# VITA-Group/mm-hand

Measured on AMD Instinct MI355X. Metric: 256x256 hand images/sec (G+D step), higher is better.
Workload: dtype f32; 1 GPU; RHD-shaped 256x256, per-GPU batch 32, fp32 (Winograd F(6x6,3x3) on the 3x3 stack), G(9 PATBlocks, ngf64)+D_PB+D_PP+L1/perceptual/GAN+Adam, --norm instance, dropout on; VGG19[:4] weights: random-init (seed 1234): NOT the reference's pretrained objective; global_batch=32, parallelism=dp1

## Files before the change

### mmhand_amd/csrc/common.h

```cpp
#pragma once
#include <hip/hip_runtime.h>
#include <cstdarg>
#include <cstdio>
#include <cstdint>
#include "../../include/mmhand_hip.h"

namespace mmh {

char* err_buf();
int fail(const char* fmt, ...);

inline int check_launch(const char* what) {
    hipError_t e = hipGetLastError();
    if (e != hipSuccess) return fail("%s: %s", what, hipGetErrorString(e));
    return 0;
}

inline hipStream_t as_stream(mmh_stream_t s) { return reinterpret_cast<hipStream_t>(s); }

inline int64_t cdiv(int64_t a, int64_t b) { return (a + b - 1) / b; }

int wino6_weights(const float* w, float* U, int Cin, int Cout, int flip_transpose, hipStream_t st);
int wino6_weights_multi(const long long* table, int n, long long total_blocks, hipStream_t st);
int wino6_input(const float* x, float* V, int B, int H, int W, int C, int reflect, int xcd, hipStream_t st);
int wino6_output(const float* M, float* y, const float* bias, int B, int H, int W, int C, int act, float* stats,
                 int fold, hipStream_t st);
int wino6_dy(const float* dy, float* Yh, int B, int H, int W, int C, hipStream_t st);
int wino6_input_normact(const float* x, float* V, int B, int H, int W, int C, int reflect, int xcd,
                        const float* scale, const float* shift, int groups, int relu, float drop_p,
                        const uint32_t* drows, hipStream_t st);
int wino6_input_dy_normbwd(const float* g, const float* x, float* V, float* Yh, int B, int H, int W, int C, int xcd,
                           int fold, const float* mean, const float* invstd, const float* gamma, const float* s1,
                           const float* s2, double count, const float* scale, const float* shift,
                           const uint32_t* drows, int groups, int relu, float drop_p, hipStream_t st);
int wino6_input_dy(const float* dy, float* V, float* Yh, int B, int H, int W, int C, int xcd, int fold,
                   hipStream_t st);
int wino6_dw(const float* dU, float* dw, int Cin, int Cout, int accumulate, hipStream_t st);
bool wgrad_lp16t_supported(const mmh_conv_desc* d);
int wgrad_lp16t_splits(const mmh_conv_desc* d);
int launch_wgrad_lp16t(const mmh_conv_desc* d, const void* x16, const void* dy16, float* slab, const void* zeros,
                       hipStream_t st);
bool dgrad_s2_halo_ok(const mmh_conv_desc* d, int dx_cs, int act);
int launch_dgrad_s2_halo(const mmh_conv_desc* d, const void* dy, const void* w, const void* bias, void* dx, int dx_cs,
                         int act, hipStream_t st);
extern int g_dgrad_s2_halo, g_dgrad_s2_dbg;
bool wgrad_s2_strip_ok(const mmh_conv_desc* d);
size_t wgrad_s2_strip_ws_bytes(const mmh_conv_desc* d);
int launch_wgrad_s2_strip(const mmh_conv_desc* d, const void* x, const void* dy, void* dw, void* ws, size_t ws_bytes,
                          int accumulate, hipStream_t st);
extern int g_wgrad_s2_strip;
bool stem_f32_ok(const mmh_conv_desc* d);
int stem_f32_stats_chunks(const mmh_conv_desc* d);
int launch_stem_f32(const mmh_conv_desc* d, const void* x, const void* w, const void* bias, void* y, int act, float* stats,
                    hipStream_t st);
extern int g_stem_f32, g_stem_f32_dbg, g_stem_f32_levels;
extern int g_stem_sparse;
extern int g_stem_sparse_flat;
void wgrad_flat_split(int Mrows, int N, int P, int& splits, int& pix_per_split);
bool wino_wgrad_dma_ok(int64_t tiles, int Cin, int Cout, int nbatch);
size_t wino_wgrad_dma_ws_bytes(int64_t tiles, int Cin, int Cout, int nbatch);
int launch_wino_wgrad_dma(const float* V, const float* Yh, int64_t tiles, int Cin, int Cout, int nbatch, float* ws, float* dU,
                          hipStream_t st);
extern int g_wino_wgrad_dma;
int launch_slab_reduce(const float* slab, float* dw, int64_t n4_total, int splits, int accumulate, int64_t n4, hipStream_t st);
bool conv_s2f_ok(const mmh_conv_desc* d, int mode);
bool conv_s1f_ok(const mmh_conv_desc* d, int mode);
int conv_s2f_stats_chunks(const mmh_conv_desc* d);
int launch_conv_s2f(const mmh_conv_desc* d, const void* x16, const void* w16, const void* bias, void* y, int y_is16, int act,
                    const void* zeros, hipStream_t st, float* stats = nullptr, int mode = 0);
bool conv_s2d_ok(const mmh_conv_desc* d, int mode);
int launch_conv_s2d(const mmh_conv_desc* d, const void* g16, const void* w16, const void* bias, void* dx, int dx_is16, int act,
                    const void* zeros, hipStream_t st);
extern int g_lp16_s2f;
extern int g_lp16_persist;
extern int g_slab_reduce_par;
extern int g_wino6_vec;
extern int g_lp16_shape;
extern int g_lp16_tap_inner;
extern int g_lp16_dbg;
extern int g_lp16_wgrad_ring;
extern int g_lp16_wgrad_s2;
extern int g_pw_v2;
extern int g_col_chunks, g_row_chunks;

}

#define MMH_REQUIRE(cond, ...)                      \
    do {                                            \
        if (!(cond)) return mmh::fail(__VA_ARGS__); \
    } while (0)
```

### mmhand_amd/csrc/conv_igemm.hip

```cpp
#include <algorithm>
#include <cstring>
#include "device_prims.h"

namespace {
using namespace mmh::dev;

typedef __bf16 bf16x4 __attribute__((ext_vector_type(4)));
typedef __bf16 bf16x2 __attribute__((ext_vector_type(2)));
typedef _Float16 f16x4 __attribute__((ext_vector_type(4)));
typedef _Float16 f16x2 __attribute__((ext_vector_type(2)));
__device__ __forceinline__ bf16x4 to_bf16x4(float4 v) {
    bf16x4 r;
    r[0] = (__bf16)v.x; r[1] = (__bf16)v.y; r[2] = (__bf16)v.z; r[3] = (__bf16)v.w;
    return r;
}
template <bool H16>
__device__ __forceinline__ bf16x4 to_lp4(float4 v) {
    if (H16) {
        f16x4 r;
        r[0] = (_Float16)v.x; r[1] = (_Float16)v.y; r[2] = (_Float16)v.z; r[3] = (_Float16)v.w;
        return __builtin_bit_cast(bf16x4, r);
    }
    return to_bf16x4(v);
}
// ... 2461 lines not shown
        wst4<BF>(Yh, (long long)(r * 4 + 2) * plane + o, f4sub(t[r][0], t[r][1]));
        wst4<BF>(Yh, (long long)(r * 4 + 3) * plane + o, f4sub(z, t[r][1]));
    }
}

__global__ void wino_dw_kernel(const float* __restrict__ dU, float* __restrict__ dw, int64_t plane4,
                               int accumulate) {
    int64_t i = (int64_t)blockIdx.x * blockDim.x + threadIdx.x;
    if (i >= plane4) return;
    const float4* in = reinterpret_cast<const float4*>(dU) + i;
    float4 u[4][4];
#pragma unroll
    for (int a = 0; a < 4; ++a)
#pragma unroll
        for (int b = 0; b < 4; ++b) u[a][b] = in[(int64_t)(a * 4 + b) * plane4];
    auto half = [](float4 v) { return make_float4(0.5f * v.x, 0.5f * v.y, 0.5f * v.z, 0.5f * v.w); };
    float4 t[3][4];
#pragma unroll
    for (int b = 0; b < 4; ++b) {
        const float4 hs = half(f4add(u[1][b], u[2][b])), hd = half(f4sub(u[1][b], u[2][b]));
        t[0][b] = f4add(u[0][b], hs);
        t[1][b] = hd;
        t[2][b] = f4add(hs, u[3][b]);
    }
    float4* out = reinterpret_cast<float4*>(dw) + i;
#pragma unroll
    for (int a = 0; a < 3; ++a) {
        const float4 hs = half(f4add(t[a][1], t[a][2])), hd = half(f4sub(t[a][1], t[a][2]));
        float4 g0 = f4add(t[a][0], hs), g1 = hd, g2 = f4add(hs, t[a][3]);
        if (accumulate) {
            g0 = f4add(g0, out[(int64_t)(a * 3 + 0) * plane4]);
            g1 = f4add(g1, out[(int64_t)(a * 3 + 1) * plane4]);
            g2 = f4add(g2, out[(int64_t)(a * 3 + 2) * plane4]);
        }
        out[(int64_t)(a * 3 + 0) * plane4] = g0;
        out[(int64_t)(a * 3 + 1) * plane4] = g1;
        out[(int64_t)(a * 3 + 2) * plane4] = g2;
    }
}

struct F2 { float x, y; };
__device__ __forceinline__ F2 operator+(F2 a, F2 b) { return {a.x + b.x, a.y + b.y}; }
__device__ __forceinline__ F2 operator-(F2 a, F2 b) { return {a.x - b.x, a.y - b.y}; }
__device__ __forceinline__ F2 operator*(float k, F2 a) { return {k * a.x, k * a.y}; }

__device__ __forceinline__ void w4_bt(const F2* in, F2* out) {
    out[0] = 4.f * in[0] - 5.f * in[2] + in[4];
    out[1] = in[3] + in[4] - 4.f * (in[1] + in[2]);
    out[2] = 4.f * (in[1] - in[2]) - in[3] + in[4];
    out[3] = 2.f * (in[3] - in[1]) - in[2] + in[4];
    out[4] = 2.f * (in[1] - in[3]) - in[2] + in[4];
    out[5] = 4.f * in[1] - 5.f * in[3] + in[5];
}
__device__ __forceinline__ void w4_at(const F2* in, F2* out) {
    const F2 a = in[1] + in[2], b = in[1] - in[2], c = in[3] + in[4], d = in[3] - in[4];
    out[0] = in[0] + a + c;
    out[1] = b + 2.f * d;
    out[2] = a + 4.f * c;
    out[3] = b + 8.f * d + in[5];
}
__device__ __forceinline__ void w4_a(const F2* in, F2* out) {
    out[0] = in[0];
    out[1] = in[0] + in[1] + in[2] + in[3];
    out[2] = in[0] - in[1] + in[2] - in[3];
    out[3] = in[0] + 2.f * in[1] + 4.f * in[2] + 8.f * in[3];
    out[4] = in[0] - 2.f * in[1] + 4.f * in[2] - 8.f * in[3];
    out[5] = in[3];
}
__device__ __forceinline__ void w4_g(const float* in, float* out) {
    out[0] = 0.25f * in[0];
    out[1] = (-1.f / 6.f) * (in[0] + in[1] + in[2]);
    out[2] = (-1.f / 6.f) * (in[0] - in[1] + in[2]);
    out[3] = (1.f / 24.f) * in[0] + (1.f / 12.f) * in[1] + (1.f / 6.f) * in[2];
    out[4] = (1.f / 24.f) * in[0] - (1.f / 12.f) * in[1] + (1.f / 6.f) * in[2];
    out[5] = in[2];
}
__device__ __forceinline__ void w4_gt(const F2* in, F2* out) {
    out[0] = 0.25f * in[0] - (1.f / 6.f) * (in[1] + in[2]) + (1.f / 24.f) * (in[3] + in[4]);
    out[1] = (1.f / 6.f) * (in[2] - in[1]) + (1.f / 12.f) * (in[3] - in[4]);
    out[2] = (1.f / 6.f) * (in[3] + in[4] - in[1] - in[2]) + in[5];
}

__global__ void wino4_weights_kernel(const float* __restrict__ w, float* __restrict__ U, int Cin, int Cout,
                                     int flip_transpose) {
    const int total = Cin * Cout;
    int i = blockIdx.x * blockDim.x + threadIdx.x;
    if (i >= total) return;
    const int ci = flip_transpose ? i % Cin : i / Cout, co = flip_transpose ? i / Cin : i - (i / Cout) * Cout;
    float g[3][3], t[6][3], col[3], o6[6];
#pragma unroll
    for (int a = 0; a < 3; ++a)
#pragma unroll
        for (int b = 0; b < 3; ++b) {
            const int ka = flip_transpose ? 2 - a : a, kb = flip_transpose ? 2 - b : b;
            g[a][b] = w[((size_t)(ka * 3 + kb) * Cin + ci) * Cout + co];
        }
#pragma unroll
    for (int b = 0; b < 3; ++b) {
        col[0] = g[0][b]; col[1] = g[1][b]; col[2] = g[2][b];
        w4_g(col, o6);
#pragma unroll
        for (int a = 0; a < 6; ++a) t[a][b] = o6[a];
    }
    const size_t plane = (size_t)Cin * Cout;
    const size_t o = flip_transpose ? (size_t)co * Cin + ci : (size_t)ci * Cout + co;
#pragma unroll
    for (int a = 0; a < 6; ++a) {
        w4_g(t[a], o6);
#pragma unroll
        for (int b = 0; b < 6; ++b) U[(size_t)(a * 6 + b) * plane + o] = o6[b];
    }
}

__global__ void wino4_input_kernel(const float* __restrict__ x, float* __restrict__ V, int B, int H, int W,
                                   int C2, int reflect, int xcd_remap) {
    const int TH = H / 4, TW = W / 4;
    const long long tiles = (long long)B * TH * TW;
    unsigned blk = blockIdx.x;
    if (xcd_remap) blk = (blk & 7u) * (gridDim.x >> 3) + (blk >> 3);
    long long i = (long long)blk * blockDim.x + threadIdx.x;
    if (i >= tiles * C2) return;
    const int c = (int)(i % C2);
    const long long tile = i / C2;
    const int tx = (int)(tile % TW), ty = (int)((tile / TW) % TH), b = (int)(tile / ((long long)TW * TH));
    const F2* xin = reinterpret_cast<const F2*>(x);
    F2 d[6][6], t[6][6], colv[6], o6[6];
#pragma unroll
    for (int r = 0; r < 6; ++r) {
        int hh = 4 * ty - 1 + r;
        bool okh = true;
        if (reflect) { hh = hh < 0 ? -hh : hh; hh = hh >= H ? 2 * (H - 1) - hh : hh; }
        else okh = hh >= 0 && hh < H;
#pragma unroll
        for (int q = 0; q < 6; ++q) {
            int ww = 4 * tx - 1 + q;
            bool ok = okh;
            if (reflect) { ww = ww < 0 ? -ww : ww; ww = ww >= W ? 2 * (W - 1) - ww : ww; }
            else ok = ok && ww >= 0 && ww < W;
            d[r][q] = ok ? xin[(((long long)b * H + hh) * W + ww) * C2 + c] : F2{0.f, 0.f};
        }
    }
#pragma unroll
    for (int q = 0; q < 6; ++q) {
#pragma unroll
        for (int r = 0; r < 6; ++r) colv[r] = d[r][q];
        w4_bt(colv, o6);
#pragma unroll
        for (int r = 0; r < 6; ++r) t[r][q] = o6[r];
    }
    const long long plane = tiles * C2;
    F2* out = reinterpret_cast<F2*>(V) + tile * C2 + c;
#pragma unroll
    for (int r = 0; r < 6; ++r) {
        w4_bt(t[r], o6);
#pragma unroll
        for (int q = 0; q < 6; ++q) out[(long long)(r * 6 + q) * plane] = o6[q];
    }
}

__global__ void wino4_output_kernel(const float* __restrict__ M, float* __restrict__ y,
                                    const float* __restrict__ bias, int B, int H, int W, int C2, int act) {
    const int TH = H / 4, TW = W / 4;
    const long long tiles = (long long)B * TH * TW;
    long long i = (long long)blockIdx.x * blockDim.x + threadIdx.x;
    if (i >= tiles * C2) return;
    const int c = (int)(i % C2);
    const long long tile = i / C2;
    const int tx = (int)(tile % TW), ty = (int)((tile / TW) % TH), b = (int)(tile / ((long long)TW * TH));
    const long long plane = tiles * C2;
    const F2* in = reinterpret_cast<const F2*>(M) + tile * C2 + c;
    F2 m[6][6], s4[4][6], colv[6], o4[4];
#pragma unroll
    for (int r = 0; r < 6; ++r)
#pragma unroll
        for (int q = 0; q < 6; ++q) m[r][q] = in[(long long)(r * 6 + q) * plane];
#pragma unroll
    for (int q = 0; q < 6; ++q) {
#pragma unroll
        for (int r = 0; r < 6; ++r) colv[r] = m[r][q];
        w4_at(colv, o4);
#pragma unroll
        for (int r = 0; r < 4; ++r) s4[r][q] = o4[r];
    }
    const F2 bv = bias ? reinterpret_cast<const F2*>(bias)[c] : F2{0.f, 0.f};
    F2* yo = reinterpret_cast<F2*>(y);
#pragma unroll
    for (int r = 0; r < 4; ++r) {
        w4_at(s4[r], o4);
#pragma unroll
        for (int q = 0; q < 4; ++q) {
            F2 v = o4[q] + bv;
            v.x = act_apply(v.x, act); v.y = act_apply(v.y, act);
            yo[(((long long)b * H + 4 * ty + r) * W + 4 * tx + q) * C2 + c] = v;
        }
    }
}

__global__ void wino4_dy_kernel(const float* __restrict__ dy, float* __restrict__ Yh, int B, int H, int W,
                                int C2) {
    const int TH = H / 4, TW = W / 4;
    const long long tiles = (long long)B * TH * TW;
    long long i = (long long)blockIdx.x * blockDim.x + threadIdx.x;
    if (i >= tiles * C2) return;
    const int c = (int)(i % C2);
    const long long tile = i / C2;
    const int tx = (int)(tile % TW), ty = (int)((tile / TW) % TH), b = (int)(tile / ((long long)TW * TH));
    const F2* in = reinterpret_cast<const F2*>(dy);
    F2 yv[4][4], t[6][4], colv[4], o6[6];
#pragma unroll
    for (int r = 0; r < 4; ++r)
#pragma unroll
        for (int q = 0; q < 4; ++q) yv[r][q] = in[(((long long)b * H + 4 * ty + r) * W + 4 * tx + q) * C2 + c];
#pragma unroll
    for (int q = 0; q < 4; ++q) {
#pragma unroll
        for (int r = 0; r < 4; ++r) colv[r] = yv[r][q];
        w4_a(colv, o6);
#pragma unroll
        for (int r = 0; r < 6; ++r) t[r][q] = o6[r];
    }
    const long long plane = tiles * C2;
    F2* out = reinterpret_cast<F2*>(Yh) + tile * C2 + c;
#pragma unroll
    for (int r = 0; r < 6; ++r) {
        w4_a(t[r], o6);
#pragma unroll
        for (int q = 0; q < 6; ++q) out[(long long)(r * 6 + q) * plane] = o6[q];
    }
}

__global__ void wino4_dw_kernel(const float* __restrict__ dU, float* __restrict__ dw, int64_t plane2,
                                int accumulate) {
    int64_t i = (int64_t)blockIdx.x * blockDim.x + threadIdx.x;
    if (i >= plane2) return;
    const F2* in = reinterpret_cast<const F2*>(dU) + i;
    F2 u[6][6], t[3][6], colv[6], o3[3];
#pragma unroll
    for (int a = 0; a < 6; ++a)
#pragma unroll
        for (int b = 0; b < 6; ++b) u[a][b] = in[(int64_t)(a * 6 + b) * plane2];
#pragma unroll
    for (int b = 0; b < 6; ++b) {
#pragma unroll
        for (int a = 0; a < 6; ++a) colv[a] = u[a][b];
        w4_gt(colv, o3);
#pragma unroll
        for (int a = 0; a < 3; ++a) t[a][b] = o3[a];
    }
    F2* out = reinterpret_cast<F2*>(dw) + i;
#pragma unroll
    for (int a = 0; a < 3; ++a) {
        w4_gt(t[a], o3);
#pragma unroll
        for (int b = 0; b < 3; ++b) {
            F2 v = o3[b];
            if (accumulate) v = v + out[(int64_t)(a * 3 + b) * plane2];
            out[(int64_t)(a * 3 + b) * plane2] = v;
        }
    }
}

template <int BN, int WM, int WN, bool NMAJOR>
int launch_batched_t(const BatchKP& bp, int nbatch, hipStream_t st) {
    constexpr size_t lds = (BM * LDA + (NMAJOR ? BN * LDA : BK * BN)) * sizeof(float) + tab_bytes(BM);
    static int ready = -1;
    if (ready != 0) ready = allow_lds(conv_igemm_batched_kernel<BN, WM, WN, NMAJOR>, lds);
    if (ready != 0) return ready;
    dim3 grid((bp.p.N + BN - 1) / BN, (bp.p.M + BM - 1) / BM, nbatch);
    hipLaunchKernelGGL((conv_igemm_batched_kernel<BN, WM, WN, NMAJOR>), grid, dim3(256), lds, st, bp);
    return mmh::check_launch("conv_igemm_batched_kernel");
}

int g_wino_bn256 = 0;
int g_wino_xcd = 1;
int g_wino_gemm_v2 = 1;
int g_wino_bf16_bk = 64;
int g_wino_bf16_occ = 3;
int g_wino_gemm_occ = 3;
int g_wino_gemm_levels = 2;
int g_wino_gemm_bn = 0;

template <int BN, int LEVELS>
static int launch_wino_gemm_t(const WinoGemmKP& p, hipStream_t st) {
    constexpr size_t lds = (size_t)(BM * LDA + BK * BN) * sizeof(float);
    static int ready = -1;
    if (ready != 0) ready = allow_lds(wino_gemm_kernel<BN, LEVELS>, lds);
    if (ready != 0) return ready;
    hipLaunchKernelGGL((wino_gemm_kernel<BN, LEVELS>), dim3(8 * p.nb), dim3(256), lds, st, p);
    return mmh::check_launch("wino_gemm_kernel");
}

static int wino_gemm_v2(const float* V, const float* U, float* Mo, long long tiles, int K, int N, hipStream_t st,
                        int nbatch, int levels, bool fold16 = false) {
    WinoGemmKP p{};
    p.A = V; p.B = U; p.C = Mo;
    p.M = (int)tiles; p.K = K; p.N = N; p.P = nbatch;
    const int bn = g_wino_gemm_bn == 64 ? 64 : (N > 64 ? 128 : 64);
    p.MT = (p.M + BM - 1) / BM;
    p.NT = (N + bn - 1) / bn;
    p.W = nbatch * p.MT * p.NT;
    p.Wx = (p.W + 7) / 8;
    const bool two = (levels ? levels : g_wino_gemm_levels) == 2 && (nbatch == 64 || fold16) && K > WINO_FOLD * BK;
    p.nb = std::min(p.Wx, 32 * g_wino_gemm_occ);
    if (two) return bn == 128 ? launch_wino_gemm_t<128, 2>(p, st) : launch_wino_gemm_t<64, 2>(p, st);
    return bn == 128 ? launch_wino_gemm_t<128, 1>(p, st) : launch_wino_gemm_t<64, 1>(p, st);
}

int wino_gemm(const float* V, const float* U, float* Mo, long long tiles, int K, int N, hipStream_t st,
              int nbatch = 16, int levels = 0) {
    MMH_REQUIRE(tiles * (long long)std::max(K, N) < (1ll << 30), "winograd: tensor too large");
    if (g_wino_gemm_v2 && K % BK == 0 && N >= 64 && N % 32 == 0) return wino_gemm_v2(V, U, Mo, tiles, K, N, st, nbatch, levels);
    BatchKP bp{};
    ConvKP& p = bp.p;
    Gather& g = p.g;
    g.src = V;
    g.src_bytes = (unsigned)((size_t)tiles * K * sizeof(float));
    g.srcH = 1; g.srcW = (int)tiles; g.src_cs = (unsigned)K;
    g.PH = 1; g.PW = (int)tiles; g.TH = 1; g.TW = 1;
    g.C4 = K / 4;
    g.ap_h = 0; g.at_h = 0; g.a0_h = 0; g.ap_w = 1; g.at_w = 0; g.a0_w = 0;
    g.shift = 0; g.reflect = 0;
    set_korder(g, p.nk, p.Kflat);
    p.w = U;
    p.w_bytes = (unsigned)((size_t)K * N * sizeof(float));
    p.out = Mo;
    p.M = (int)tiles; p.N = N;
    p.wCin = K; p.wCout = N;
    p.KW_true = 1; p.kh0 = 0; p.kw0 = 0; p.tstep = 1;
    p.OH = 1; p.OW = (int)tiles; p.o_p = 1;
    p.out_cs = (unsigned)N; p.out_linear = 1;
    p.act = MMH_ACT_NONE;
    bp.src_bs = tiles * K; bp.w_bs = (long long)K * N; bp.out_bs = tiles * N;
    {
        const int bn = (N % 256 == 0 && g_wino_bn256) ? 256 : 128;
        const int gx = (N + bn - 1) / bn, gy = (p.M + BM - 1) / BM;
        p.xcd_remap = (g_conv_xcd && gx > 1 && gy >= 8) ? 1 : 0;
    }
    if (N % 256 == 0 && g_wino_bn256) return launch_batched_t<256, 2, 2, false>(bp, nbatch, st);
    if (N > 64) return launch_batched_t<128, 2, 2, false>(bp, nbatch, st);
    if (N > 32) return launch_batched_t<64, 2, 2, false>(bp, nbatch, st);
    return launch_batched_t<32, 4, 1, false>(bp, nbatch, st);
}

int g_wgrad_slots = 768;
int g_wgrad_bn256 = 1;
int g_wino_wgrad_v2 = 1;
int g_wino_wgrad_occ = 3;
int g_wgrad_xcd = 1;
int g_wino_wgrad_bn256 = 0;
int g_wino_wgrad_slots = 2304;

int wgrad_splits(int Mrows, int N, int P) {
    const int bn = (g_wgrad_bn256 && N % 256 == 0) ? 256 : 128;
    const int tiles = ((Mrows + BM - 1) / BM) * ((N + bn - 1) / bn);
    const int slots = g_wgrad_slots;
    int max_splits = P / (8 * BK);
    if (max_splits > 256) max_splits = 256;
    if (max_splits < 1) max_splits = 1;
    int best = 1;
    double best_eff = 0.0;
    for (int s = 1; s <= max_splits; ++s) {
        const int blocks = tiles * s;
        const int rounds = (blocks + slots - 1) / slots;
        const double eff = (double)blocks / ((double)rounds * slots);
        if (eff > best_eff + 1e-9) { best_eff = eff; best = s; }
        if (blocks >= 4 * slots) break;
    }
    return best;
}

int wgrad_pix_per_split(int P, int splits, int step) { return (int)(mmh::cdiv(mmh::cdiv(P, splits), step) * step); }

int g_wgrad_dbuf = 0;

template <int BN, int WM, int WN, bool DBUF>
int launch_wgrad_t(const WgradKP& p, int splits, hipStream_t st) {
    constexpr size_t lds = (DBUF ? 2 : 1) * (BK * LDW + BK * BN) * sizeof(float);
    static int ready = -1;
    if (ready != 0) ready = allow_lds(conv_wgrad_kernel<BN, WM, WN, DBUF>, lds);
    if (ready != 0) return ready;
    dim3 grid((p.N + BN - 1) / BN, (p.Mrows + BM - 1) / BM, splits);
    hipLaunchKernelGGL((conv_wgrad_kernel<BN, WM, WN, DBUF>), grid, dim3(256), lds, st, p);
    return mmh::check_launch("conv_wgrad_kernel");
}

template <int BN, int WM, int WN>
int launch_wgrad_bf16_t(const WgradKP& p, int splits, hipStream_t st) {
    constexpr size_t lds = (size_t)2 * BKP * LDT * 2;
    dim3 grid((p.N + BN - 1) / BN, (p.Mrows + BM - 1) / BM, splits);
    if (p.x16) {
        static int ready16 = -1;
        if (ready16 != 0) ready16 = allow_lds(conv_wgrad_bf16_kernel<BN, WM, WN, true>, lds);
        if (ready16 != 0) return ready16;
        hipLaunchKernelGGL((conv_wgrad_bf16_kernel<BN, WM, WN, true>), grid, dim3(256), lds, st, p);
        return mmh::check_launch("conv_wgrad_bf16_kernel");
    }
    static int ready = -1;
    if (ready != 0) ready = allow_lds(conv_wgrad_bf16_kernel<BN, WM, WN, false>, lds);
    if (ready != 0) return ready;
    hipLaunchKernelGGL((conv_wgrad_bf16_kernel<BN, WM, WN, false>), grid, dim3(256), lds, st, p);
    return mmh::check_launch("conv_wgrad_bf16_kernel");
}

template <int BN, int WM, int WN>
int launch_wgrad_grid_t(const WgradKP& p, dim3 grid, hipStream_t st) {
    constexpr size_t lds = (BK * LDW + BK * BN) * sizeof(float);
    static int ready = -1;
    if (ready != 0) ready = allow_lds(conv_wgrad_kernel<BN, WM, WN, false>, lds);
    if (ready != 0) return ready;
    hipLaunchKernelGGL((conv_wgrad_kernel<BN, WM, WN, false>), grid, dim3(256), lds, st, p);
    return mmh::check_launch("conv_wgrad_kernel");
}

size_t wgrad_ws(const mmh_conv_desc* d) {
    const int Mrows = d->kh * d->kw * d->Cin;
    const int P = d->B * d->Ho * d->Wo;
    const size_t generic = (size_t)wgrad_splits(Mrows, d->Cout, P) * Mrows * d->Cout * sizeof(float);
    return mmh::wgrad_s2_strip_ok(d) ? std::max(generic, mmh::wgrad_s2_strip_ws_bytes(d)) : generic;
}

int do_wgrad(const mmh_conv_desc* d, const void* x, const void* dy, void* dw, void* ws,
             size_t ws_bytes, int accumulate, hipStream_t st, bool x16 = false, bool dy16 = false) {
    MMH_REQUIRE(!(x16 || dy16) || is16(d->dtype), "wgrad: 16-bit operands need a 16-bit dtype");
    MMH_REQUIRE(x16 == dy16, "wgrad: io16 must be 0 (both tensors fp32) or 3 (both 16-bit)");
    if (!x16 && mmh::wgrad_s2_strip_ok(d)) return mmh::launch_wgrad_s2_strip(d, x, dy, dw, ws, ws_bytes, accumulate, st);
    WgradKP p{};
    p.g = fwd_gather(d, x);
    p.g.chunk_major = 0;
    p.x16 = x16 ? 1 : 0;
    p.dy16 = dy16 ? 1 : 0;
    if (x16) p.g.src_bytes /= 2;
    p.dy = static_cast<const float*>(dy);
    p.dy_bytes = (unsigned)((size_t)d->B * d->Ho * d->Wo * d->y_cs * (dy16 ? 2 : sizeof(float)));
    p.dy_cs = (unsigned)d->y_cs;
    p.Mrows = d->kh * d->kw * d->Cin;
    p.N = d->Cout;
    p.P = d->B * d->Ho * d->Wo;
    const int splits = wgrad_splits(p.Mrows, p.N, p.P);
    MMH_REQUIRE(ws_bytes >= (size_t)splits * p.Mrows * p.N * sizeof(float),
                "wgrad workspace too small: %zu < %zu", ws_bytes,
                (size_t)splits * p.Mrows * p.N * sizeof(float));
    p.slab = static_cast<float*>(ws);
    const bool bf16 = is16(d->dtype);
    p.h16 = d->dtype == MMH_FP16;
    p.pix_per_split = wgrad_pix_per_split(p.P, splits, bf16 ? BKP : BK);
    p.dbg = g_conv_dbg;
    p.nsplit = splits;
    int rc;
    if (bf16) {
        if (p.N > 64) rc = launch_wgrad_bf16_t<128, 2, 2>(p, splits, st);
        else if (p.N > 32) rc = launch_wgrad_bf16_t<64, 2, 2>(p, splits, st);
        else rc = launch_wgrad_bf16_t<32, 4, 1>(p, splits, st);
    } else if (g_wgrad_bn256 && p.N % 256 == 0) rc = launch_wgrad_t<256, 2, 2, false>(p, splits, st);
    else if (p.N > 64) rc = g_wgrad_dbuf ? launch_wgrad_t<128, 2, 2, true>(p, splits, st)
                                    : launch_wgrad_t<128, 2, 2, false>(p, splits, st);
    else if (p.N > 32) rc = launch_wgrad_t<64, 2, 2, false>(p, splits, st);
    else rc = launch_wgrad_t<32, 4, 1, false>(p, splits, st);
    if (rc) return rc;
    const int64_t n4 = (int64_t)p.Mrows * p.N / 4;
    return mmh::launch_slab_reduce(p.slab, static_cast<float*>(dw), n4, splits, accumulate, n4, st);
}

struct OptionEntry { const char* name; int* value; };
const OptionEntry* option_table(int* count) {
    static const OptionEntry table[] = {
        {"conv_dbuf", &g_conv_dbuf},
        {"conv_dbg", &g_conv_dbg},
        {"conv_cw", &g_conv_cw},
        {"conv_bn256", &g_conv_bn256},
        {"conv_levels", &g_conv_levels},
        {"dgrad_levels", &g_dgrad_levels},
        {"wino_bn256", &g_wino_bn256},
        {"conv_xcd", &g_conv_xcd},
        {"conv_xcd1", &g_conv_xcd1},
        {"conv_tall", &g_conv_tall},
        {"wgrad_slots", &g_wgrad_slots},
        {"wgrad_dbuf", &g_wgrad_dbuf},
        {"wgrad_bn256", &g_wgrad_bn256},
        {"wgrad_xcd", &g_wgrad_xcd},
        {"wino_wgrad_v2", &g_wino_wgrad_v2},
        {"wino_wgrad_occ", &g_wino_wgrad_occ},
        {"wino_gemm_v2", &g_wino_gemm_v2},
        {"wino_xcd", &g_wino_xcd},
        {"dgrad_s2_multi", &g_dgrad_s2_multi},
        {"wino6_vec", &mmh::g_wino6_vec},
        {"lp16_shape", &mmh::g_lp16_shape},
        {"lp16_s2f", &mmh::g_lp16_s2f},
        {"lp16_persist", &mmh::g_lp16_persist},
        {"lp16_tap_inner", &mmh::g_lp16_tap_inner},
        {"pw_v2", &mmh::g_pw_v2},
        {"col_chunks", &mmh::g_col_chunks},
        {"row_chunks", &mmh::g_row_chunks},
        {"dgrad_s2_halo", &mmh::g_dgrad_s2_halo},
        {"wgrad_s2_strip", &mmh::g_wgrad_s2_strip},
        {"stem_f32", &mmh::g_stem_f32},
        {"wino_wgrad_dma", &mmh::g_wino_wgrad_dma},
        {"stem_f32_dbg", &mmh::g_stem_f32_dbg},
        {"slab_reduce_par", &mmh::g_slab_reduce_par},
        {"dgrad_s2_dbg", &mmh::g_dgrad_s2_dbg},
        {"lp16_dbg", &mmh::g_lp16_dbg},
        {"lp16_wgrad_ring", &mmh::g_lp16_wgrad_ring},
        {"lp16_wgrad_s2", &mmh::g_lp16_wgrad_s2},
        {"border_bn64", &g_border_bn64},
        {"wino_gemm_occ", &g_wino_gemm_occ},
        {"wino_gemm_levels", &g_wino_gemm_levels},
        {"wino_gemm_bn", &g_wino_gemm_bn},
        {"wino_bf16_occ", &g_wino_bf16_occ},
        {"wino_bf16_bk", &g_wino_bf16_bk},
        {"wino_wgrad_bn256", &g_wino_wgrad_bn256},
        {"wino_wgrad_slots", &g_wino_wgrad_slots},
        {"stem_sparse", &mmh::g_stem_sparse},
        {"stem_sparse_flat", &mmh::g_stem_sparse_flat},
    };
    *count = (int)(sizeof(table) / sizeof(table[0]));
    return table;
}
const OptionEntry* find_option(const char* key) {
    int n = 0;
    const OptionEntry* t = option_table(&n);
    for (int i = 0; i < n; ++i)
        if (!strcmp(key, t[i].name)) return &t[i];
    return nullptr;
}

}

namespace mmh {
void wgrad_flat_split(int Mrows, int N, int P, int& splits, int& pix_per_split) {
    splits = wgrad_splits(Mrows, N, P);
    pix_per_split = wgrad_pix_per_split(P, splits, BK);
}
}

extern "C" {

int mmh_set_option(const char* key, int value) {
    MMH_REQUIRE(key != nullptr, "mmh_set_option: NULL key");
    const OptionEntry* e = find_option(key);
    if (!e) return mmh::fail("mmh_set_option: unknown key '%s'", key);
    if (e->value == &g_conv_levels) { g_conv_levels = value == 2 ? 2 : 1; mmh::g_stem_f32_levels = g_conv_levels; return 0; }
    if (e->value == &g_dgrad_levels) { g_dgrad_levels = value == 2 ? 2 : 1; return 0; }
    if (e->value == &mmh::g_col_chunks || e->value == &mmh::g_row_chunks)
        MMH_REQUIRE(value > 0, "mmh_set_option: '%s' needs a value > 0, got %d", key, value);
    *e->value = value;
    return 0;
}

int mmh_get_option(const char* key, int* value) {
    MMH_REQUIRE(key != nullptr && value != nullptr, "mmh_get_option: NULL key or value");
    const OptionEntry* e = find_option(key);
    if (!e) return mmh::fail("mmh_get_option: unknown key '%s'", key);
    *value = *e->value;
    return 0;
}

const char* mmh_option_key(int index) {
    int n = 0;
    const OptionEntry* t = option_table(&n);
    return index >= 0 && index < n ? t[index].name : nullptr;
}

int mmh_conv2d_fprop(const mmh_conv_desc* d, const void* x, const void* w, const void* bias,
                     void* y, int act, mmh_stream_t s) {
    if (int rc = validate(d)) return rc;
    MMH_REQUIRE(x && w && y, "mmh_conv2d_fprop: NULL buffer");
    return do_fprop(d, x, w, bias, y, act, mmh::as_stream(s));
}

int mmh_conv2d_fprop_rect(const mmh_conv_desc* d, int pad_h, int pad_w, const void* x, const void* w, const void* bias,
                          void* y, int act, mmh_stream_t s) {
    MMH_REQUIRE(d != nullptr, "conv desc is NULL");
    MMH_REQUIRE(d->dtype == MMH_F32 && d->pad_mode == MMH_PAD_ZERO, "mmh_conv2d_fprop_rect: fp32 and zero padding only");
    MMH_REQUIRE(d->Cin > 0 && d->Cout > 0 && d->Cin % 4 == 0 && d->Cout % 4 == 0, "Cin/Cout must be multiples of 4 (%d,%d)", d->Cin,
                d->Cout);
    MMH_REQUIRE(d->x_cs % 4 == 0 && d->y_cs % 4 == 0 && d->x_cs >= d->Cin && d->y_cs >= d->Cout,
                "bad channel strides x_cs=%d y_cs=%d", d->x_cs, d->y_cs);
    MMH_REQUIRE(d->stride == 1 || d->stride == 2, "stride must be 1 or 2 (%d)", d->stride);
    MMH_REQUIRE(d->B >= 1 && d->H >= 1 && d->W >= 1 && d->kh >= 1 && d->kw >= 1 && pad_h >= 0 && pad_w >= 0 && pad_h < d->kh &&
                    pad_w < d->kw && d->H + 2 * pad_h >= d->kh && d->W + 2 * pad_w >= d->kw,
                "mmh_conv2d_fprop_rect: bad kernel/pad (%dx%d, pad %d,%d on %dx%d)", d->kh, d->kw, pad_h, pad_w, d->H, d->W);
    MMH_REQUIRE(d->Ho == (d->H + 2 * pad_h - d->kh) / d->stride + 1 && d->Wo == (d->W + 2 * pad_w - d->kw) / d->stride + 1,
                "Ho/Wo inconsistent with H,W,k,s,pad_h,pad_w");
    MMH_REQUIRE((int64_t)d->B * (d->H + 2 * pad_h) * (d->W + 2 * pad_w) * (int64_t)d->x_cs < (1ll << 30) &&
                    (int64_t)d->B * d->Ho * d->Wo * (int64_t)d->y_cs < (1ll << 30) &&
                    (int64_t)d->kh * d->kw * d->Cin * d->Cout < (1ll << 30),
                "tensor too large for 32-bit byte offsets (4 GiB per buffer)");
    MMH_REQUIRE(x && w && y, "mmh_conv2d_fprop_rect: NULL buffer");
    const int pads[2] = {pad_h, pad_w};
    return do_fprop(d, x, w, bias, y, act, mmh::as_stream(s), nullptr, pads);
}

int mmh_conv2d_fprop_stats_chunks(const mmh_conv_desc* d) { return d ? fprop_stats_chunks(d) : 0; }

int mmh_conv2d_fprop_stats(const mmh_conv_desc* d, const void* x, const void* w, const void* bias, void* y,
                           void* stats, mmh_stream_t s) {
    if (int rc = validate(d)) return rc;
    MMH_REQUIRE(x && w && y && stats, "mmh_conv2d_fprop_stats: NULL buffer");
    MMH_REQUIRE(fprop_stats_chunks(d) > 0, "mmh_conv2d_fprop_stats: needs fp32 and B*Ho*Wo %% 128 == 0");
    return do_fprop(d, x, w, bias, y, MMH_ACT_NONE, mmh::as_stream(s), static_cast<float*>(stats));
}

int mmh_conv2d_dgrad(const mmh_conv_desc* d, const void* dy, const void* w, void* dx, int dx_cs,
                     mmh_stream_t s) {
    if (int rc = validate(d)) return rc;
    MMH_REQUIRE(dy && w && dx, "mmh_conv2d_dgrad: NULL buffer");
    MMH_REQUIRE(dx_cs % 4 == 0 && dx_cs >= d->Cin, "mmh_conv2d_dgrad: bad dx_cs=%d", dx_cs);
    return do_dgrad(d, dy, w, nullptr, dx, dx_cs, MMH_ACT_NONE, mmh::as_stream(s));
}

static int wino_planes(int tile) { return (tile + 2) * (tile + 2); }
static bool wino_tile_ok(int tile) { return tile == 2 || tile == 4 || tile == 6; }
static bool wino_hw_ok(int H, int W, int tile) {
    return tile == 6 ? (H >= 4 && W >= 4) : (H >= tile + 2 && W >= tile + 2 && H % tile == 0 && W % tile == 0);
}
static long long wino_tiles(int B, int H, int W, int tile) {
    return (long long)B * ((H + tile - 1) / tile) * ((W + tile - 1) / tile);
}

static bool wino_dtype_ok(int dtype, int tile) { return dtype == MMH_F32 || (is16(dtype) && tile == 2); }

int mmh_wino_weights(const void* w, int Cin, int Cout, int flip_transpose, int tile, int dtype, void* U,
                     mmh_stream_t s) {
    MMH_REQUIRE(w && U && Cin > 0 && Cout > 0 && wino_tile_ok(tile) && wino_dtype_ok(dtype, tile),
                "mmh_wino_weights: bad arguments (tile 2 | 4 | 6; bf16 needs tile 2)");
    const dim3 grid((Cin * Cout + 255) / 256);
    if (tile == 6)
        return mmh::wino6_weights(static_cast<const float*>(w), static_cast<float*>(U), Cin, Cout, flip_transpose,
                                  mmh::as_stream(s));
    if (tile == 4)
        hipLaunchKernelGGL(wino4_weights_kernel, grid, dim3(256), 0, mmh::as_stream(s),
                           static_cast<const float*>(w), static_cast<float*>(U), Cin, Cout, flip_transpose);
    else if (dtype == MMH_FP16)
        hipLaunchKernelGGL(wino_weights_kernel<2>, grid, dim3(256), 0, mmh::as_stream(s),
                           static_cast<const float*>(w), U, Cin, Cout, flip_transpose);
    else if (dtype == MMH_BF16)
        hipLaunchKernelGGL(wino_weights_kernel<1>, grid, dim3(256), 0, mmh::as_stream(s),
                           static_cast<const float*>(w), U, Cin, Cout, flip_transpose);
    else
        hipLaunchKernelGGL(wino_weights_kernel<0>, grid, dim3(256), 0, mmh::as_stream(s),
                           static_cast<const float*>(w), U, Cin, Cout, flip_transpose);
    return mmh::check_launch("wino_weights_kernel");
}

static bool wino_fold_ok(int H, int W) { return H >= 6 && W >= 6 && (H + 1) % 6 >= 2 && (W + 1) % 6 >= 2; }

int mmh_wino_weights_multi(const void* table, int n, int64_t total_blocks, mmh_stream_t s) {
    MMH_REQUIRE(table && n > 0 && total_blocks > 0 && total_blocks < (1ll << 31), "mmh_wino_weights_multi: bad arguments");
    return mmh::wino6_weights_multi(static_cast<const long long*>(table), n, total_blocks, mmh::as_stream(s));
}

int mmh_wino_input(const void* x, int B, int H, int W, int C, int reflect, int tile, int dtype, void* V,
                   mmh_stream_t s) {
    MMH_REQUIRE(x && V && B > 0 && wino_tile_ok(tile) && wino_hw_ok(H, W, tile) && C % 4 == 0 &&
                    wino_dtype_ok(dtype, tile) && reflect >= 0 && reflect <= 2,
                "mmh_wino_input: bad arguments");
    MMH_REQUIRE(reflect != 2 || (tile == 6 && dtype == MMH_F32 && wino_fold_ok(H, W)),
                "mmh_wino_input: pad mode 2 (padded-domain dgrad) needs tile 6, fp32, (H+1) %% 6 >= 2, (W+1) %% 6 >= 2");
    const long long tiles = wino_tiles(B, H, W, tile);
    if (tile == 6)
        return mmh::wino6_input(static_cast<const float*>(x), static_cast<float*>(V), B, H, W, C, reflect, g_wino_xcd,
                                mmh::as_stream(s));
    if (tile == 4) {
        const long long total = tiles * (C / 2);
        const unsigned nblk = (unsigned)((total + 255) / 256);
        hipLaunchKernelGGL(wino4_input_kernel, dim3(nblk), dim3(256), 0, mmh::as_stream(s),
                           static_cast<const float*>(x), static_cast<float*>(V), B, H, W, C / 2, reflect,
                           (g_wino_xcd && nblk % 8 == 0 && nblk >= 64) ? 1 : 0);
    } else {
        const long long total = tiles * (C / 4);
        const dim3 grid((unsigned)((total + 255) / 256));
        if (dtype == MMH_FP16)
            hipLaunchKernelGGL(wino_input_kernel<2>, grid, dim3(256), 0, mmh::as_stream(s),
                               static_cast<const float*>(x), V, B, H, W, C / 4, reflect);
        else if (dtype == MMH_BF16)
            hipLaunchKernelGGL(wino_input_kernel<1>, grid, dim3(256), 0, mmh::as_stream(s),
                               static_cast<const float*>(x), V, B, H, W, C / 4, reflect);
        else
            hipLaunchKernelGGL(wino_input_kernel<0>, grid, dim3(256), 0, mmh::as_stream(s),
                               static_cast<const float*>(x), V, B, H, W, C / 4, reflect);
    }
    return mmh::check_launch("wino_input_kernel");
}

int mmh_wino_input_dy(const void* dy, int B, int H, int W, int C, int tile, int dtype, void* V, void* Yh,
                      int fold, mmh_stream_t s) {
    MMH_REQUIRE(dy && V && Yh && B > 0 && tile == 6 && dtype == MMH_F32 && wino_hw_ok(H, W, tile) && C % 4 == 0,
                "mmh_wino_input_dy: needs tile 6, fp32");
    MMH_REQUIRE(!fold || (wino_fold_ok(H, W) && (H + 7) / 6 == (H + 5) / 6 && (W + 7) / 6 == (W + 5) / 6),
                "mmh_wino_input_dy: fold needs (H+1) %% 6 >= 2 and ceil((H+2)/6) == ceil(H/6) (W alike)");
    return mmh::wino6_input_dy(static_cast<const float*>(dy), static_cast<float*>(V), static_cast<float*>(Yh), B, H, W,
                               C, g_wino_xcd, fold ? 1 : 0, mmh::as_stream(s));
}

int mmh_wino_input_normact(const void* x, int B, int H, int W, int C, int reflect, void* V, const void* scale,
                           const void* shift, int groups, int relu, float drop_p, const void* drows,
                           mmh_stream_t s) {
    MMH_REQUIRE(x && V && scale && shift && B > 0 && wino_hw_ok(H, W, 6) && C % 8 == 0 && reflect >= 0 && reflect <= 1 &&
                    (groups == 1 || groups == B) && drop_p >= 0.f && drop_p < 1.f && (drop_p == 0.f) == (drows == nullptr) &&
                    (drop_p == 0.f || relu),
                "mmh_wino_input_normact: bad arguments (tile 6, fp32, C %% 8 == 0, groups 1 | B, dropout rows iff p > 0)");
    MMH_REQUIRE((long long)B * H * W * C < (1ll << 31), "mmh_wino_input_normact: 32-bit element offsets (numel < 2^31)");
    return mmh::wino6_input_normact(static_cast<const float*>(x), static_cast<float*>(V), B, H, W, C, reflect,
                                    g_wino_xcd, static_cast<const float*>(scale), static_cast<const float*>(shift),
                                    groups, relu, drop_p, static_cast<const uint32_t*>(drows), mmh::as_stream(s));
}

int mmh_wino_input_dy_normbwd(const void* g, const void* x, int B, int H, int W, int C, void* V, void* Yh, int fold,
                              const void* mean, const void* invstd, const void* gamma, const void* s1,
                              const void* s2, double count, const void* scale, const void* shift,
                              const void* drows, int groups, int relu, float drop_p, mmh_stream_t s) {
    MMH_REQUIRE(g && x && V && Yh && mean && invstd && s1 && s2 && scale && shift && B > 0 && wino_hw_ok(H, W, 6) &&
                    C % 8 == 0 && count > 0 && (groups == 1 || groups == B) && drop_p >= 0.f && drop_p < 1.f &&
                    (drop_p == 0.f) == (drows == nullptr),
                "mmh_wino_input_dy_normbwd: bad arguments (tile 6, fp32, C %% 8 == 0, groups 1 | B)");
    MMH_REQUIRE((long long)B * H * W * C < (1ll << 31), "mmh_wino_input_dy_normbwd: 32-bit element offsets (numel < 2^31)");
    MMH_REQUIRE(!fold || (wino_fold_ok(H, W) && (H + 7) / 6 == (H + 5) / 6 && (W + 7) / 6 == (W + 5) / 6),
                "mmh_wino_input_dy_normbwd: fold needs (H+1) %% 6 >= 2 and ceil((H+2)/6) == ceil(H/6) (W alike)");
    return mmh::wino6_input_dy_normbwd(
        static_cast<const float*>(g), static_cast<const float*>(x), static_cast<float*>(V), static_cast<float*>(Yh), B,
        H, W, C, g_wino_xcd, fold ? 1 : 0, static_cast<const float*>(mean), static_cast<const float*>(invstd),
        static_cast<const float*>(gamma), static_cast<const float*>(s1), static_cast<const float*>(s2), count,
        static_cast<const float*>(scale), static_cast<const float*>(shift), static_cast<const uint32_t*>(drows), groups,
        relu, drop_p, mmh::as_stream(s));
}

int mmh_wino_dy(const void* dy, int B, int H, int W, int C, int tile, int dtype, void* Yh, mmh_stream_t s) {
    MMH_REQUIRE(dy && Yh && B > 0 && wino_tile_ok(tile) && wino_hw_ok(H, W, tile) && C % 4 == 0 &&
                    wino_dtype_ok(dtype, tile),
                "mmh_wino_dy: bad arguments");
    const long long tiles = wino_tiles(B, H, W, tile);
    if (tile == 6)
        return mmh::wino6_dy(static_cast<const float*>(dy), static_cast<float*>(Yh), B, H, W, C, mmh::as_stream(s));
    if (tile == 4) {
        const long long total = tiles * (C / 2);
        hipLaunchKernelGGL(wino4_dy_kernel, dim3((unsigned)((total + 255) / 256)), dim3(256), 0, mmh::as_stream(s),
                           static_cast<const float*>(dy), static_cast<float*>(Yh), B, H, W, C / 2);
    } else {
        const long long total = tiles * (C / 4);
        const dim3 grid((unsigned)((total + 255) / 256));
        if (dtype == MMH_FP16)
            hipLaunchKernelGGL(wino_dy_kernel<2>, grid, dim3(256), 0, mmh::as_stream(s),
                               static_cast<const float*>(dy), Yh, B, H, W, C / 4);
        else if (dtype == MMH_BF16)
            hipLaunchKernelGGL(wino_dy_kernel<1>, grid, dim3(256), 0, mmh::as_stream(s),
                               static_cast<const float*>(dy), Yh, B, H, W, C / 4);
        else
            hipLaunchKernelGGL(wino_dy_kernel<0>, grid, dim3(256), 0, mmh::as_stream(s),
                               static_cast<const float*>(dy), Yh, B, H, W, C / 4);
    }
    return mmh::check_launch("wino_dy_kernel");
}

static int wino_gemm_bf16(const void* V, const void* U, void* Mo, long long tiles, int K, int N, int nbatch, int h16,
                          hipStream_t st) {
    MMH_REQUIRE(K % BK16 == 0 && N % 32 == 0, "mmh_wino_gemm (bf16): needs K %% 64 == 0 and N %% 32 == 0");
    MMH_REQUIRE(tiles * (long long)std::max(K, N) < (1ll << 30), "winograd: tensor too large");
    WinoGemmBfKP p{};
    p.A = static_cast<const __bf16*>(V); p.B = static_cast<const __bf16*>(U); p.C = static_cast<__bf16*>(Mo);
    p.M = (int)tiles; p.K = K; p.N = N; p.P = nbatch;
    p.h16 = h16;
    p.MT = (p.M + BM - 1) / BM;
    p.NT = (N + 127) / 128;
    p.W = nbatch * p.MT * p.NT;
    p.Wx = (p.W + 7) / 8;
    if (g_wino_bf16_bk == 128 && K % 128 == 0) {
        p.nb = std::min(p.Wx, 32 * 2);
        constexpr size_t lds = (size_t)(2 * BM * (128 + 8)) * sizeof(__bf16);
        static int ready = -1;
        if (ready != 0) ready = allow_lds(wino_gemm_bf16_kernel<128, false>, lds) | allow_lds(wino_gemm_bf16_kernel<128, true>, lds);
        if (ready != 0) return ready;
        if (h16) hipLaunchKernelGGL((wino_gemm_bf16_kernel<128, true>), dim3(8 * p.nb), dim3(256), lds, st, p);
        else hipLaunchKernelGGL((wino_gemm_bf16_kernel<128, false>), dim3(8 * p.nb), dim3(256), lds, st, p);
    } else {
        p.nb = std::min(p.Wx, 32 * g_wino_bf16_occ);
        constexpr size_t lds = (size_t)(2 * BM * (64 + 8)) * sizeof(__bf16);
        static int ready = -1;
        if (ready != 0) ready = allow_lds(wino_gemm_bf16_kernel<64, false>, lds) | allow_lds(wino_gemm_bf16_kernel<64, true>, lds);
        if (ready != 0) return ready;
        if (h16) hipLaunchKernelGGL((wino_gemm_bf16_kernel<64, true>), dim3(8 * p.nb), dim3(256), lds, st, p);
        else hipLaunchKernelGGL((wino_gemm_bf16_kernel<64, false>), dim3(8 * p.nb), dim3(256), lds, st, p);
    }
    return mmh::check_launch("wino_gemm_bf16_kernel");
}

int mmh_wino_gemm(const void* V, const void* U, void* M, int64_t tiles, int K, int N, int nbatch, int dtype,
                  mmh_stream_t s) {
    MMH_REQUIRE(V && U && M && tiles > 0 && K % 32 == 0 && N % 4 == 0 && nbatch > 0 &&
                    (dtype == MMH_F32 || is16(dtype)),
                "mmh_wino_gemm: bad arguments");
    if (is16(dtype)) return wino_gemm_bf16(V, U, M, tiles, K, N, nbatch, dtype == MMH_FP16, mmh::as_stream(s));
    return wino_gemm(static_cast<const float*>(V), static_cast<const float*>(U), static_cast<float*>(M), tiles,
                     K, N, mmh::as_stream(s), nbatch);
}

int mmh_wino_gemm_levels(const void* V, const void* U, void* M, int64_t tiles, int K, int N, int nbatch, int levels,
                         mmh_stream_t s) {
    MMH_REQUIRE(V && U && M && tiles > 0 && K % 32 == 0 && N % 4 == 0 && nbatch > 0 && (levels == 1 || levels == 2),
                "mmh_wino_gemm_levels: bad arguments (fp32; levels 1 | 2)");
    return wino_gemm(static_cast<const float*>(V), static_cast<const float*>(U), static_cast<float*>(M), tiles, K, N,
// ... 252 lines not shown
```

Baseline: 130.1 images/s.

## Add persistent DMA-staged Winograd batched GEMM kernel with 256x256 tiles

```diff
diff --git a/mmhand_amd/csrc/common.h b/mmhand_amd/csrc/common.h
--- a/mmhand_amd/csrc/common.h
+++ b/mmhand_amd/csrc/common.h
@@ -62,6 +62,10 @@
 int launch_wino_wgrad_dma(const float* V, const float* Yh, int64_t tiles, int Cin, int Cout, int nbatch, float* ws, float* dU,
                           hipStream_t st);
 extern int g_wino_wgrad_dma;
+bool wino_gemm_dma_ok(int64_t tiles, int K, int N, int nbatch, bool two);
+int launch_wino_gemm_dma(const float* V, const float* U, float* Mo, int64_t tiles, int K, int N, int nbatch, bool two,
+                         hipStream_t st);
+extern int g_wino_gemm_dma, g_wino_gemm_dma_grid;
 int launch_slab_reduce(const float* slab, float* dw, int64_t n4_total, int splits, int accumulate, int64_t n4, hipStream_t st);
 bool conv_s2f_ok(const mmh_conv_desc* d, int mode);
 bool conv_s1f_ok(const mmh_conv_desc* d, int mode);
diff --git a/mmhand_amd/csrc/conv_igemm.hip b/mmhand_amd/csrc/conv_igemm.hip
--- a/mmhand_amd/csrc/conv_igemm.hip
+++ b/mmhand_amd/csrc/conv_igemm.hip
@@ -2787,6 +2787,7 @@
     p.Wx = (p.W + 7) / 8;
     const bool two = (levels ? levels : g_wino_gemm_levels) == 2 && (nbatch == 64 || fold16) && K > WINO_FOLD * BK;
     p.nb = std::min(p.Wx, 32 * g_wino_gemm_occ);
+    if (mmh::wino_gemm_dma_ok(tiles, K, N, nbatch, two)) return mmh::launch_wino_gemm_dma(V, U, Mo, tiles, K, N, nbatch, two, st);
     if (two) return bn == 128 ? launch_wino_gemm_t<128, 2>(p, st) : launch_wino_gemm_t<64, 2>(p, st);
     return bn == 128 ? launch_wino_gemm_t<128, 1>(p, st) : launch_wino_gemm_t<64, 1>(p, st);
 }
@@ -2980,6 +2981,8 @@
         {"wgrad_s2_strip", &mmh::g_wgrad_s2_strip},
         {"stem_f32", &mmh::g_stem_f32},
         {"wino_wgrad_dma", &mmh::g_wino_wgrad_dma},
+        {"wino_gemm_dma", &mmh::g_wino_gemm_dma},
+        {"wino_gemm_dma_grid", &mmh::g_wino_gemm_dma_grid},
         {"stem_f32_dbg", &mmh::g_stem_f32_dbg},
         {"slab_reduce_par", &mmh::g_slab_reduce_par},
         {"dgrad_s2_dbg", &mmh::g_dgrad_s2_dbg},
diff --git a/mmhand_amd/csrc/wino_gemm_dma.hip b/mmhand_amd/csrc/wino_gemm_dma.hip
--- /dev/null
+++ b/mmhand_amd/csrc/wino_gemm_dma.hip
@@ -0,0 +1,237 @@
+#include <algorithm>
+#include "device_prims.h"
+
+namespace mmh { int g_wino_gemm_dma = 1, g_wino_gemm_dma_grid = 0; }
+
+namespace {
+using namespace mmh::dev;
+
+constexpr int NT = 512;
+constexpr int BMR = 256, BNC = 256;
+constexpr int KS = 32;
+constexpr int A_B = BMR * KS * 4;
+constexpr int B_B = KS * BNC * 4;
+constexpr int ST_B = A_B + B_B;
+constexpr int LDS_B = 2 * ST_B;
+constexpr int AR = A_B / (NT * 16), BR = B_B / (NT * 16);
+constexpr int CUS = 256;
+
+struct WinoGemmDmaKP {
+    const float* A;
+    const float* B;
+    float* C;
+    int M, K, N, P;
+    int pairs;
+    int NTc;
+    int S;
+    int nst;
+};
+
+struct Item { int pl, m0, n0, np; };
+
+template <int LEVELS>
+__global__ void __launch_bounds__(NT, 1) wino_gemm_dma_kernel(const WinoGemmDmaKP p) {
+    extern __shared__ __attribute__((aligned(1024))) char smem[];
+    const int tid = threadIdx.x;
+    const int lane = tid & 63, wave = __builtin_amdgcn_readfirstlane(tid >> 6);
+    const int l31 = lane & 31, h = lane >> 5;
+    const int wm = wave >> 2, wn = wave & 3;
+    const unsigned lds0 = lds_addr_of(smem);
+    const unsigned wdst = __builtin_amdgcn_readfirstlane(lds0 + (unsigned)wave * 1024u);
+
+    const int G = (int)gridDim.x;
+    const int L = (G & 7) ? (int)blockIdx.x : (int)((blockIdx.x & 7) * (G >> 3) + (blockIdx.x >> 3));
+    const int s0 = (int)((long long)L * p.S / G), s1 = (int)((long long)(L + 1) * p.S / G);
+    if (s0 >= s1) return;
+    const int per_plane = p.pairs * p.NTc, per_rb = 4 * p.NTc;
+    const int rb_last = (p.pairs - 1) >> 2;
+    auto item_at = [&](int s) {
+        Item it;
+        it.pl = s / per_plane;
+        const int x = s - it.pl * per_plane;
+        int rb = x / per_rb, np = 4;
+        if (rb >= rb_last) { rb = rb_last; np = p.pairs - 4 * rb_last; }
+        const int y = x - rb * per_rb, col = y / np, pr = y - col * np;
+        it.m0 = rb * BMR + pr * 64;
+        it.n0 = col * BNC;
+        it.np = min(np - pr, s1 - s);
+        return it;
+    };
+
+    unsigned a_off[AR], b_off[BR];
+#pragma unroll
+    for (int i = 0; i < BR; ++i) {
+        const int u = i * NT + tid;
+        b_off[i] = (unsigned)((u >> 6) * p.N * 4 + (u & 63) * 16);
+    }
+    const float* la = nullptr;
+    const float* lb = nullptr;
+    int ls = s0, lks = 0, lnp = 0;
+    auto setup_load = [&]() {
+        const Item it = item_at(ls);
+        la = p.A + (size_t)it.pl * p.M * p.K;
+        lb = p.B + (size_t)it.pl * p.K * p.N + it.n0;
+        lnp = it.np;
+#pragma unroll
+        for (int k = 0; k < AR; ++k) {
+            const int u = k * NT + tid;
+            const int R = u >> 3, chunk = (u & 7) ^ ((R >> 1) & 7);
+            const int row = it.m0 + 64 * ((R >> 5) & 3) + 32 * (R >> 7) + (R & 31);
+            a_off[k] = (unsigned)min(row, p.M - 1) * (unsigned)p.K * 4u + (unsigned)chunk * 16u;
+        }
+    };
+    auto issue_next = [&](int slot) {
+        if (ls >= s1) return;
+        const unsigned dst = wdst + (unsigned)(slot * ST_B);
+        const float* const va = la + lks * KS;
+        const float* const ub = lb + (size_t)lks * KS * p.N;
+#pragma unroll
+        for (int k = 0; k < AR; ++k)
+            if (((2 * k + wm) & 3) < lnp) dma16_s(va, a_off[k], dst + (unsigned)(k * NT * 16));
+#pragma unroll
+        for (int k = 0; k < BR; ++k) dma16_s(ub, b_off[k], dst + (unsigned)(A_B + k * NT * 16));
+        if (++lks == p.nst) {
+            lks = 0;
+            ls += lnp;
+            if (ls < s1) setup_load();
+        }
+    };
+
+    f32x16 acc[4][2];
+#pragma unroll
+    for (int i = 0; i < 4; ++i)
+#pragma unroll
+        for (int j = 0; j < 2; ++j)
+#pragma unroll
+            for (int e = 0; e < 16; ++e) acc[i][j][e] = 0.f;
+
+    const int sw = (l31 >> 1) & 7;
+    const unsigned a_lane = lds0 + (unsigned)((128 * wm + l31) * 128);
+    const unsigned b_lane = lds0 + (unsigned)(A_B + 4 * h * BNC * 4 + (64 * wn + l31) * 4);
+    unsigned a_kg[4];
+#pragma unroll
+    for (int kg = 0; kg < 4; ++kg) a_kg[kg] = a_lane + (unsigned)(((2 * kg + h) ^ sw) * 16);
+
+    setup_load();
+    issue_next(0);
+    int slot = 0;
+    for (int cs = s0; cs < s1;) {
+        const Item it = item_at(cs);
+        cs += it.np;
+        const int nact = __builtin_amdgcn_readfirstlane(max(0, min(it.np, (p.M - it.m0 - 32 * wm + 63) >> 6)));
+        float* const o = p.C + ((size_t)it.pl * p.M + it.m0 + 32 * wm) * p.N + it.n0 + 64 * wn;
+        const unsigned o_lane = (unsigned)(4 * h * p.N + l31);
+        const int rows_left = p.M - (it.m0 + 32 * wm + 4 * h);
+        for (int ks = 0; ks < p.nst; ++ks) {
+            asm volatile("" ::: "memory");
+            __builtin_amdgcn_s_waitcnt(0x0070);
+            __builtin_amdgcn_s_barrier();
+            asm volatile("" ::: "memory");
+            if (wm == 0) issue_next(slot ^ 1);
+            unsigned bb = b_lane + (unsigned)(slot * ST_B);
+            unsigned ab[4];
+#pragma unroll
+            for (int kg = 0; kg < 4; ++kg) ab[kg] = a_kg[kg] + (unsigned)(slot * ST_B);
+            asm volatile("" : "+v"(bb), "+v"(ab[0]), "+v"(ab[1]), "+v"(ab[2]), "+v"(ab[3]));
+            f32x4 av[2];
+            float bv[2][2][4];
+            auto frags = [&](int t, int buf) {
+                const int i = t >> 2, kg = t & 3;
+                av[buf] = lds_f4(ab[kg], i * 4096);
+#pragma unroll
+                for (int j = 0; j < 2; ++j)
+#pragma unroll
+                    for (int e = 0; e < 4; ++e) bv[buf][j][e] = lds_f(bb, (kg * 8 + e) * BNC * 4 + j * 128);
+            };
+            frags(0, 0);
+            f32x16 part[2];
+#pragma unroll
+            for (int t = 0; t < 16; ++t) {
+                const int i = t >> 2, kg = t & 3, buf = t & 1;
+                if (t + 1 < 16) frags(t + 1, buf ^ 1);
+                if (__builtin_expect(i < nact, 1)) {
+#pragma unroll
+                    for (int e = 0; e < 4; ++e)
+#pragma unroll
+                        for (int j = 0; j < 2; ++j) {
+                            if constexpr (LEVELS == 2)
+                                part[j] = __builtin_amdgcn_mfma_f32_32x32x2f32(av[buf][e], bv[buf][j][e],
+                                                                               (kg == 0 && e == 0) ? f32x16{} : part[j], 0, 0, 0);
+                            else
+                                acc[i][j] = __builtin_amdgcn_mfma_f32_32x32x2f32(av[buf][e], bv[buf][j][e], acc[i][j], 0, 0, 0);
+                        }
+                    if constexpr (LEVELS == 2) {
+                        if (kg == 3) {
+#pragma unroll
+                            for (int j = 0; j < 2; ++j)
+#pragma unroll
+                                for (int e = 0; e < 16; ++e) acc[i][j][e] += part[j][e];
+                        }
+                    }
+                }
+                if (t == 7 && wm != 0) issue_next(slot ^ 1);
+            }
+            slot ^= 1;
+        }
+        unsigned ol = o_lane;
+        asm volatile("" : "+v"(ol));
+#pragma unroll
+        for (int i = 0; i < 4; ++i)
+            if (i < nact) {
+#pragma unroll
+                for (int e = 0; e < 16; ++e) {
+                    const int dr = 64 * i + (e & 3) + 8 * (e >> 2);
+                    if (dr < rows_left) {
+                        float* const c = o + (size_t)dr * p.N + ol;
+                        c[0] = acc[i][0][e];
+                        c[32] = acc[i][1][e];
+                    }
+                }
+#pragma unroll
+                for (int j = 0; j < 2; ++j)
+#pragma unroll
+                    for (int e = 0; e < 16; ++e) acc[i][j][e] = 0.f;
+            }
+    }
+}
+
+template <int LEVELS>
+int launch_t(const WinoGemmDmaKP& p, int grid, hipStream_t st) {
+    static int ready = -1;
+    if (ready != 0) {
+        hipError_t e = hipFuncSetAttribute(reinterpret_cast<const void*>(wino_gemm_dma_kernel<LEVELS>),
+                                           hipFuncAttributeMaxDynamicSharedMemorySize, LDS_B);
+        if (e != hipSuccess) return mmh::fail("wino_gemm_dma: %s", hipGetErrorString(e));
+        ready = 0;
+    }
+    hipLaunchKernelGGL((wino_gemm_dma_kernel<LEVELS>), dim3(grid), dim3(NT), LDS_B, st, p);
+    return mmh::check_launch("wino_gemm_dma_kernel");
+}
+
+}
+
+namespace mmh {
+
+bool wino_gemm_dma_ok(int64_t tiles, int K, int N, int nbatch, bool two) {
+    static const struct { int tiles, K, N; bool two; } tie[] = {{3872, 256, 512, false}, {3872, 512, 512, false}};
+    if (nbatch == 64 && g_wino_gemm_dma != 2)
+        for (const auto& t : tie)
+            if (tiles == t.tiles && K == t.K && N == t.N && two == t.two) return false;
+    return g_wino_gemm_dma && K > 0 && K % KS == 0 && N > 0 && N % BNC == 0 && tiles > 0 && nbatch > 0 &&
+           tiles * (int64_t)std::max(K, N) < (1ll << 29) && (int64_t)nbatch * ((tiles + 63) / 64) * (N / BNC) < (1ll << 30);
+}
+
+int launch_wino_gemm_dma(const float* V, const float* U, float* Mo, int64_t tiles, int K, int N, int nbatch, bool two,
+                         hipStream_t st) {
+    WinoGemmDmaKP p{};
+    p.A = V; p.B = U; p.C = Mo;
+    p.M = (int)tiles; p.K = K; p.N = N; p.P = nbatch;
+    p.pairs = (p.M + 63) / 64; p.NTc = N / BNC;
+    p.S = nbatch * p.pairs * p.NTc;
+    p.nst = K / KS;
+    int grid = std::min(CUS, (p.S + 3) / 4);
+    if (g_wino_gemm_dma_grid > 0) grid = std::min(grid, g_wino_gemm_dma_grid);
+    return two ? launch_t<2>(p, grid, st) : launch_t<1>(p, grid, st);
+}
+
+}
```

After: 130.6 images/s (median of 6 runs). Within noise of the previous version (+0.4%).
